# ClashLuke/LocAtE

Measured on AMD Instinct MI355X. Metric: images/sec (G+D step) 64x64 bs=64, higher is better.
Workload: dtype f32 (contractions fp32-faithful on the matrix cores: 2 x scaled fp16 operand pieces / 3 MFMAs per slice where the operand's largest magnitude comes with it, else 3 x bf16 pieces / 6 MFMAs; fp32 accumulate); 1 GPU; LocAtE G+D step, 64x64 RGB, batch 64 per GPU (the fp32 variant - the reference's own precision - of BASELINE.json configs[1]: 64x64 RGB bs 64), self/feature attention at 16x16 and 64x64, random-init weights; global_batch=64, image_size=64, parallelism=dp1, launch=hipGraph replay, G-step generator pass on a second stream

## Files before the change

locate_amd/csrc/conv.hip:

```cpp
#include "igemm.h"



struct PackBatch {
    PackArgs ph[4];
};

__device__ __forceinline__ void pack_tables(const PackArgs& a, int k) {
    int* koff = reinterpret_cast<int*>(a.out + (size_t)a.rows * a.ld);
    unsigned char* ktap = reinterpret_cast<unsigned char*>(koff + a.rows);
    const int T = a.TH * a.TW;
    int off = 0, tap = 31;
    if (k < a.K && T > 0) {
        const int c = k / T, t = k - c * T;
        const int th = t / a.TW, tw = t - th * a.TW;
        off = 4 * (c * a.gHW + (a.dy0 + a.dys * th) * a.gW + a.dx0 + a.dxs * tw - a.dmin);
        tap = t;
    }
    koff[k] = off;
    ktap[k] = (unsigned char)tap;
}

__device__ __forceinline__ void pack_publish_absmax(float m, const PackArgs* phases, int nphase, float* red) {
    m = wave_max(m);
// ... 1704 lines not shown
                                 int scale_group_batch, int scale_stride, const float* bias, float* gx, int64_t gx_bs,
                                 void* workspace, void* counters, int precision, const void* gy_absmax, const void* act_epilogue,
                                 void* stream) {
    const ConvGeom g = make_geom(geom);
    if (int e = geom_check(g, "locate_conv_dgrad")) return e;
    LOCATE_REQUIRE(gy && panel && gx, "locate_conv_dgrad: null pointer");
    return run_igemm(g, 1, gy, gy_bs, panel, scale, scale_group_batch, scale_stride, bias, gx, gx_bs,
                     static_cast<float*>(workspace), static_cast<unsigned*>(counters), precision, static_cast<const unsigned*>(gy_absmax),
                     as_stream(stream), "locate_conv_dgrad", static_cast<const LocateActEpilogue*>(act_epilogue));
}

#define WG_BK 32

struct WgParams {
    const float* x;
    const float* gy;
    float* slab;
    long long x_bs, gy_bs;
    unsigned x_bytes;
    int B, C, H, W, M, OH, OW, KH, KW, stride, pad_h, pad_w;
    int R;
    int N;
    int chunk;
    int zper, Ng;
    unsigned q_mul, ow_mul;
    int q_s1, q_s2, ow_s1, ow_s2;
    int gscale_bg, gscale_stride;
    float* direct_out;
    const float* w_ref;
    const float* inv_scale;
    double* partial;
    const unsigned* x_absmax;
    const unsigned* g_absmax;
};


template <int WGM, int WGN, int TM, int TN>
__device__ __forceinline__ void wgrad_epilogue(const WgParams& p, f32x16 (&acc)[TM][TN], int r0, int m0, int wm, int wn, int lane,
                                               int wid, int tid) {
    const int lrow = lane >> 5, lcol = lane & 31;
    __shared__ double red[4];
    const bool direct = p.direct_out != nullptr;
    float* dst = direct ? p.direct_out : p.slab + (long long)blockIdx.z * p.M * p.R;
    const float sc = (direct && p.inv_scale && p.gscale_bg == 0) ? p.inv_scale[0] : 1.0f;
    double dot = 0.0;
    const bool want_dot = direct && p.w_ref != nullptr;
#pragma unroll
    for (int j = 0; j < TN; ++j) {
        const int r = r0 + (wn * TN + j) * 32 + lcol;
        const bool r_ok = r < p.R;
#pragma unroll
        for (int i = 0; i < TM; ++i) {
            float wref[16];
#pragma unroll
            for (int e = 0; e < 16; ++e) {
                const int m = m0 + (wm * TM + i) * 32 + (e & 3) + 8 * (e >> 2) + 4 * lrow;
                const bool ok = want_dot && r_ok && m < p.M;
                const float* wp_ = ok ? p.w_ref + (long long)m * p.R + r : p.gy;
                wref[e] = ok ? *wp_ : 0.0f;
            }
            float part = 0.0f;
#pragma unroll
            for (int e = 0; e < 16; ++e) {
                const int m = m0 + (wm * TM + i) * 32 + (e & 3) + 8 * (e >> 2) + 4 * lrow;
                const float v = acc[i][j][e];
                part = fmaf(v, wref[e], part);
                if (r_ok && m < p.M) dst[(long long)m * p.R + r] = v * sc;
            }
            dot += (double)part;
        }
    }
    if (direct && p.partial) {
        dot = wave_sum_d(dot);
        if (lane == 0) red[wid] = dot;
        __syncthreads();
        if (tid == 0) p.partial[blockIdx.y * gridDim.x + blockIdx.x] = (red[0] + red[1]) + (red[2] + red[3]);
    }
}

template <int WGM, int WGN, int TM, int TN>
__global__ void __launch_bounds__(256) conv_wgrad_kernel(const WgParams p) {
    constexpr int BM = WGM * TM * 32;
    constexpr int BR = WGN * TN * 32;
    constexpr int G_PT = WG_BK * BM / 256;
    constexpr int X_PT = WG_BK * BR / 256;
    static_assert(WGM * WGN == 4, "four waves");

    __shared__ float Gs[2][WG_BK][BM + 1];
    __shared__ float Xs[2][WG_BK][BR + 1];
    __shared__ int rt_off[BR];
    __shared__ signed char rt_dy[BR], rt_dx[BR];

    const int tid = threadIdx.x, lane = tid & 63, wid = tid >> 6;
    const int wm = wid / WGN, wn = wid % WGN;
    const int r0 = blockIdx.x * BR, m0 = blockIdx.y * BM;
    const int taps = p.KH * p.KW;
    for (int i = tid; i < BR; i += 256) {
        const int r = r0 + i;
        if (r < p.R) {
            const int c = r / taps, t = r - c * taps;
            const int kh = t / p.KW, kw = t - kh * p.KW;
            rt_dy[i] = (signed char)(kh - p.pad_h);
            rt_dx[i] = (signed char)(kw - p.pad_w);
            rt_off[i] = c * p.H * p.W + (kh - p.pad_h) * p.W + (kw - p.pad_w);
        } else {
            rt_dy[i] = rt_dx[i] = 0;
            rt_off[i] = -2147483647 - 1;
        }
    }
    __syncthreads();

    f32x16 acc[TM][TN];
#pragma unroll
    for (int i = 0; i < TM; ++i)
#pragma unroll
        for (int j = 0; j < TN; ++j)
#pragma unroll
            for (int r = 0; r < 16; ++r) acc[i][j][r] = 0.0f;

    const int zgrp = (int)blockIdx.z / p.zper;
    const int n_begin = zgrp * p.Ng + ((int)blockIdx.z - zgrp * p.zper) * p.chunk;
    int n_end = n_begin + p.chunk;
    if (n_end > (zgrp + 1) * p.Ng) n_end = (zgrp + 1) * p.Ng;
    const int nl = tid & 31, sub = tid >> 5;
// ... 54 lines not shown
    auto store_tiles = [&](int buf) {
#pragma unroll
        for (int i = 0; i < G_PT; ++i) Gs[buf][nl][sub + 8 * i] = ((gmask >> i) & 1u) ? greg[i] * gsc : 0.0f;
#pragma unroll
        for (int i = 0; i < X_PT; ++i) Xs[buf][nl][sub + 8 * i] = ((xmask >> i) & 1u) ? xreg[i] : 0.0f;
    };

    const int nsteps = (n_end - n_begin + WG_BK - 1) / WG_BK;
    const int lrow = lane >> 5, lcol = lane & 31;
    if (nsteps > 0) {
        load_tiles(n_begin);
        store_tiles(0);
    }
    __syncthreads();
    for (int s = 0; s < nsteps; ++s) {
        const int buf = s & 1;
        if (s + 1 < nsteps) load_tiles(n_begin + (s + 1) * WG_BK);
#pragma unroll
        for (int k2 = 0; k2 < WG_BK / 2; ++k2) {
            float a[TM], b[TN];
#pragma unroll
            for (int i = 0; i < TM; ++i) a[i] = Gs[buf][k2 * 2 + lrow][(wm * TM + i) * 32 + lcol];
#pragma unroll
            for (int j = 0; j < TN; ++j) b[j] = Xs[buf][k2 * 2 + lrow][(wn * TN + j) * 32 + lcol];
#pragma unroll
            for (int i = 0; i < TM; ++i)
#pragma unroll
                for (int j = 0; j < TN; ++j) acc[i][j] = __builtin_amdgcn_mfma_f32_32x32x2f32(a[i], b[j], acc[i][j], 0, 0, 0);
        }
        if (s + 1 < nsteps) store_tiles(buf ^ 1);
        __syncthreads();
    }

    wgrad_epilogue<WGM, WGN, TM, TN>(p, acc, r0, m0, wm, wn, lane, wid, tid);
}

#define WB_BK 16
#define WB_PITCH 8

template <int WGM, int WGN, int TM, int TN, int NP>
__global__ void __launch_bounds__(256, (WGM * TM > 4 ? 2 : 3)) conv_wgrad_bx6_kernel(const WgParams p) {
    constexpr int BM = WGM * TM * 32;
    constexpr int BR = WGN * TN * 32;
    constexpr int G_PT = BM / 32;
    constexpr int X_PT = BR / 32;
    static_assert(WGM * WGN == 4, "four waves");

    constexpr int NPL = NP == 4 ? 1 : NP;
    __shared__ unsigned Gs[2][NPL][NP == 4 ? 1 : BM][WB_PITCH];
    __shared__ unsigned Xs[2][NPL][NP == 4 ? 1 : BR][WB_PITCH];
    __shared__ __attribute__((aligned(16))) unsigned short G8[2][NP == 4 ? BM : 1][8];
    __shared__ __attribute__((aligned(16))) unsigned short X8[2][NP == 4 ? BR : 1][8];

    const int tid = threadIdx.x, lane = tid & 63, wid = tid >> 6;
    const int wm = wid / WGN, wn = wid % WGN;
    const int r0 = blockIdx.x * BR, m0 = blockIdx.y * BM;
    const int taps = p.KH * p.KW;
    const int np = tid & 7, sub = tid >> 3;
    const int Q = p.OH * p.OW;

    int xoff[X_PT], xdy[X_PT], xdx[X_PT];
#pragma unroll
    for (int i = 0; i < X_PT; ++i) {
        const int r = r0 + sub + 32 * i;
        if (r < p.R) {
            const int c = r / taps, t = r - c * taps;
            const int kh = t / p.KW, kw = t - kh * p.KW;
            xdy[i] = kh - p.pad_h;
            xdx[i] = kw - p.pad_w;
            xoff[i] = 4 * (c * p.H * p.W + xdy[i] * p.W + xdx[i]);
        } else {
            xdy[i] = -(1 << 20);
            xdx[i] = 0;
            xoff[i] = 0;
        }
    }
    const __amdgpu_buffer_rsrc_t xrsrc = __builtin_amdgcn_make_buffer_rsrc(const_cast<float*>(p.x), 0, (int)p.x_bytes, 0x00020000);

    f32x16 acc[TM][TN];
#pragma unroll
    for (int i = 0; i < TM; ++i)
#pragma unroll
        for (int j = 0; j < TN; ++j)
#pragma unroll
            for (int r = 0; r < 16; ++r) acc[i][j][r] = 0.0f;

    const int zgrp = (int)blockIdx.z / p.zper;
    const int n_begin = zgrp * p.Ng + ((int)blockIdx.z - zgrp * p.zper) * p.chunk;
    int n_end = n_begin + p.chunk;
    if (n_end > (zgrp + 1) * p.Ng) n_end = (zgrp + 1) * p.Ng;

    float gs0 = 1.0f, gs1 = 1.0f, gs2 = 1.0f, gs3 = 1.0f, gsc = 1.0f;
    if (p.gscale_bg > 0) {
        const int ng = p.B / p.gscale_bg;
        gs0 = p.inv_scale[0];
        gs1 = ng > 1 ? p.inv_scale[p.gscale_stride] : 1.0f;
        gs2 = ng > 2 ? p.inv_scale[2 * p.gscale_stride] : 1.0f;
        gs3 = ng > 3 ? p.inv_scale[3 * p.gscale_stride] : 1.0f;
    }

    float g_scale = 1.0f, x_scale = 1.0f, g_unscale = 1.0f, x_unscale = 1.0f;
    if constexpr (NP == 2) {
        const float gmax = __uint_as_float(absmax_read(p.g_absmax)) * fmaxf(fmaxf(gs0, gs1), fmaxf(gs2, gs3));
        const int kg_ = f16_scale_exp(__float_as_uint(gmax) + (p.gscale_bg > 0 ? 0x00800000u : 0u));
        const int kx_ = f16_scale_exp(absmax_read(p.x_absmax));
        g_scale = pow2f(kg_); g_unscale = pow2f(-kg_);
        x_scale = pow2f(kx_); x_unscale = pow2f(-kx_);
    }
    if constexpr (NP == 4) {
        const float gmax = __uint_as_float(absmax_read(p.g_absmax)) * fmaxf(fmaxf(gs0, gs1), fmaxf(gs2, gs3));
        const int kg_ = f8_scale_exp(__float_as_uint(gmax) + (p.gscale_bg > 0 ? 0x00800000u : 0u));
        const int kx_ = f8_scale_exp(absmax_read(p.x_absmax));
        g_scale = pow2f(kg_); g_unscale = pow2f(-kg_);
        x_scale = pow2f(kx_); x_unscale = pow2f(-kx_);
    }
    auto q8_pair = [](float v0, float v1) { return (unsigned short)(__builtin_amdgcn_cvt_pk_fp8_f32(v0, v1, 0, false) & 0xffff); };
    auto h8 = [](int row, int pair) { return ((((pair >> 2) ^ (row >> 4)) & 1) << 2) | (pair & 3); };

    float2 greg[G_PT], xreg[X_PT];
    auto load_tiles = [&](int nb) {
        const int n = nb + 2 * np;
        const bool ok = n < n_end;
        const int nn = ok ? n : 0;
        const int b = fastdiv(nn, p.q_mul, p.q_s1, p.q_s2), q = nn - b * Q;
        const int oh = fastdiv(q, p.ow_mul, p.ow_s1, p.ow_s2), ow = q - oh * p.OW;
        const float* gp = p.gy + (long long)b * p.gy_bs + q;
        if (p.gscale_bg > 0) {
            const int bg = p.gscale_bg;
            gsc = gs0;
            gsc = b >= bg ? gs1 : gsc;
            gsc = b >= 2 * bg ? gs2 : gsc;
            gsc = b >= 3 * bg ? gs3 : gsc;
        }
#pragma unroll
        for (int i = 0; i < G_PT; ++i) {
            const int m = m0 + sub + 32 * i;
            const bool v = ok && m < p.M;
            const float2 t = *reinterpret_cast<const float2*>(gp + (v ? (long long)m * Q : 0));
            greg[i] = v ? t : make_float2(0.0f, 0.0f);
        }
        const int iy0 = oh * p.stride, ix0 = ow * p.stride;
        const unsigned base = (unsigned)(4 * ((long long)b * p.x_bs + (long long)iy0 * p.W + ix0));
#pragma unroll
        for (int i = 0; i < X_PT; ++i) {
            const bool vy = ok && (unsigned)(iy0 + xdy[i]) < (unsigned)p.H;
            const bool v0 = vy && (unsigned)(ix0 + xdx[i]) < (unsigned)p.W;
            const bool v1 = vy && (unsigned)(ix0 + p.stride + xdx[i]) < (unsigned)p.W;
            const unsigned o = base + (unsigned)xoff[i];
            xreg[i].x = __builtin_bit_cast(float, __builtin_amdgcn_raw_buffer_load_b32(xrsrc, (int)(v0 ? o : 0x80000000u), 0, 0));
            xreg[i].y = __builtin_bit_cast(float, __builtin_amdgcn_raw_buffer_load_b32(xrsrc, (int)(v1 ? o + 4u * (unsigned)p.stride : 0x80000000u), 0, 0));
        }
    };
    const int wcol = (((np >> 2) ^ ((sub >> 3) & 1)) << 2) | (np & 3);
    auto store_tiles = [&](int buf) {
#pragma unroll
        for (int i = 0; i < G_PT; ++i) {
            if constexpr (NP == 2) {
                unsigned h, l;
                split2_f16_pair(greg[i].x * gsc * g_scale, greg[i].y * gsc * g_scale, h, l);
                Gs[buf][0][sub + 32 * i][wcol] = h;
                Gs[buf][NP - 1][sub + 32 * i][wcol] = l;
            } else if constexpr (NP == 3) {
                unsigned h, m, l;
                split3_trunc_pair(greg[i].x * gsc, greg[i].y * gsc, h, m, l);
                Gs[buf][0][sub + 32 * i][wcol] = h;
                Gs[buf][NP - 2][sub + 32 * i][wcol] = m;
                Gs[buf][NP - 1][sub + 32 * i][wcol] = l;
            } else if constexpr (NP == 4) {
                G8[buf][sub + 32 * i][h8(sub + 32 * i, np)] = q8_pair(greg[i].x * gsc * g_scale, greg[i].y * gsc * g_scale);
            } else {
                Gs[buf][0][sub + 32 * i][wcol] = round_bf16_pair(greg[i].x * gsc, greg[i].y * gsc);
            }
        }
#pragma unroll
        for (int i = 0; i < X_PT; ++i) {
            if constexpr (NP == 2) {
                unsigned h, l;
                split2_f16_pair(xreg[i].x * x_scale, xreg[i].y * x_scale, h, l);
                Xs[buf][0][sub + 32 * i][wcol] = h;
                Xs[buf][NP - 1][sub + 32 * i][wcol] = l;
            } else if constexpr (NP == 3) {
                unsigned h, m, l;
                split3_trunc_pair(xreg[i].x, xreg[i].y, h, m, l);
                Xs[buf][0][sub + 32 * i][wcol] = h;
                Xs[buf][NP - 2][sub + 32 * i][wcol] = m;
                Xs[buf][NP - 1][sub + 32 * i][wcol] = l;
            } else if constexpr (NP == 4) {
                X8[buf][sub + 32 * i][h8(sub + 32 * i, np)] = q8_pair(xreg[i].x * x_scale, xreg[i].y * x_scale);
            } else {
                Xs[buf][0][sub + 32 * i][wcol] = round_bf16_pair(xreg[i].x, xreg[i].y);
            }
        }
    };

    const int nsteps = (n_end - n_begin + WB_BK - 1) / WB_BK;
    const int lrow = lane >> 5, lcol = lane & 31;
    const int rhalf = lrow ^ ((lcol >> 3) & 1);
    if (nsteps > 0) {
        load_tiles(n_begin);
        store_tiles(0);
        load_tiles(n_begin + WB_BK);
    }
    __syncthreads();
    constexpr int PROD = NP == 3 ? 6 : (NP == 2 ? 3 : 1);
    constexpr int NMF = TM * TN * PROD, HALF = NMF / 2;
    using frag_t = typename std::conditional<NP == 2, f16x8, bf16x8>::type;
    for (int s = 0; s < nsteps; ++s) {
        const int buf = s & 1;
        frag_t a[TM][NPL], b[TN][NPL];
        long a8[TM], b8[TN];
        if constexpr (NP == 4) {
            const int half8 = (lrow ^ (lcol >> 4)) & 1;
#pragma unroll
            for (int i = 0; i < TM; ++i) a8[i] = *reinterpret_cast<const long*>(&G8[buf][(wm * TM + i) * 32 + lcol][half8 * 4]);
#pragma unroll
            for (int j = 0; j < TN; ++j) b8[j] = *reinterpret_cast<const long*>(&X8[buf][(wn * TN + j) * 32 + lcol][half8 * 4]);
        } else {
#pragma unroll
            for (int i = 0; i < TM; ++i)
#pragma unroll
                for (int q = 0; q < NPL; ++q) a[i][q] = *reinterpret_cast<const frag_t*>(&Gs[buf][q][(wm * TM + i) * 32 + lcol][rhalf * 4]);
#pragma unroll
            for (int j = 0; j < TN; ++j)
#pragma unroll
                for (int q = 0; q < NPL; ++q) b[j][q] = *reinterpret_cast<const frag_t*>(&Xs[buf][q][(wn * TN + j) * 32 + lcol][rhalf * 4]);
        }
        auto mfmas = [&](int lo, int hi) {
#pragma unroll
            for (int i = 0; i < TM; ++i)
#pragma unroll
                for (int j = 0; j < TN; ++j) {
                    const int base = (i * TN + j) * PROD;
                    if constexpr (NP == 2) {
                        if (base + 0 >= lo && base + 0 < hi) acc[i][j] = __builtin_amdgcn_mfma_f32_32x32x16_f16(a[i][1], b[j][0], acc[i][j], 0, 0, 0);
                        if (base + 1 >= lo && base + 1 < hi) acc[i][j] = __builtin_amdgcn_mfma_f32_32x32x16_f16(a[i][0], b[j][1], acc[i][j], 0, 0, 0);
                        if (base + 2 >= lo && base + 2 < hi) acc[i][j] = __builtin_amdgcn_mfma_f32_32x32x16_f16(a[i][0], b[j][0], acc[i][j], 0, 0, 0);
                    } else if constexpr (NP == 3) {
                        if (base + 0 >= lo && base + 0 < hi) acc[i][j] = __builtin_amdgcn_mfma_f32_32x32x16_bf16(a[i][NP - 1], b[j][0], acc[i][j], 0, 0, 0);
                        if (base + 1 >= lo && base + 1 < hi) acc[i][j] = __builtin_amdgcn_mfma_f32_32x32x16_bf16(a[i][0], b[j][NP - 1], acc[i][j], 0, 0, 0);
                        if (base + 2 >= lo && base + 2 < hi) acc[i][j] = __builtin_amdgcn_mfma_f32_32x32x16_bf16(a[i][NP - 2], b[j][NP - 2], acc[i][j], 0, 0, 0);
                        if (base + 3 >= lo && base + 3 < hi) acc[i][j] = __builtin_amdgcn_mfma_f32_32x32x16_bf16(a[i][NP - 2], b[j][0], acc[i][j], 0, 0, 0);
                        if (base + 4 >= lo && base + 4 < hi) acc[i][j] = __builtin_amdgcn_mfma_f32_32x32x16_bf16(a[i][0], b[j][NP - 2], acc[i][j], 0, 0, 0);
                        if (base + 5 >= lo && base + 5 < hi) acc[i][j] = __builtin_amdgcn_mfma_f32_32x32x16_bf16(a[i][0], b[j][0], acc[i][j], 0, 0, 0);
                    } else if constexpr (NP == 4) {
                        if (base >= lo && base < hi) acc[i][j] = __builtin_amdgcn_mfma_f32_32x32x16_fp8_fp8(a8[i], b8[j], acc[i][j], 0, 0, 0);
                    } else {
                        if (base >= lo && base < hi) acc[i][j] = __builtin_amdgcn_mfma_f32_32x32x16_bf16(a[i][0], b[j][0], acc[i][j], 0, 0, 0);
                    }
                }
        };
        __builtin_amdgcn_sched_barrier(0);
        mfmas(0, HALF);
        __builtin_amdgcn_sched_barrier(0);
        store_tiles(buf ^ 1);
        load_tiles(n_begin + (s + 2) * WB_BK);
        __builtin_amdgcn_sched_barrier(0);
        mfmas(HALF, NMF);
        __syncthreads();
    }
    if constexpr (NP == 2 || NP == 4) {
#pragma unroll
        for (int i = 0; i < TM; ++i)
#pragma unroll
            for (int j = 0; j < TN; ++j)
#pragma unroll
                for (int r = 0; r < 16; ++r) acc[i][j][r] = (acc[i][j][r] * g_unscale) * x_unscale;
    }
    wgrad_epilogue<WGM, WGN, TM, TN>(p, acc, r0, m0, wm, wn, lane, wid, tid);
}

template <int V>
__device__ __forceinline__ void slab_load(const float* p, float (&v)[V]) {
    if constexpr (V == 4) { const float4 t = *reinterpret_cast<const float4*>(p); v[0] = t.x; v[1] = t.y; v[2] = t.z; v[3] = t.w; }
    else v[0] = *p;
}

template <int ZP, int V>
__device__ __forceinline__ void slab_reduce_groups(const float* __restrict__ slab, float* __restrict__ out, int64_t n, int nsplit,
                                                   const float* __restrict__ w_ref, double* __restrict__ partial, int bid, int nblocks,
                                                   int groups, int zper, float* zbuf, double* gscratch) {
    float (*gzsum)[ZP][256 / ZP][V] = reinterpret_cast<float (*)[ZP][256 / ZP][V]>(zbuf);
    constexpr int TPB = 256 / ZP, EPB = TPB * V;
    const int ex = threadIdx.x % TPB, ez = threadIdx.x / TPB;
    const int64_t stride = (int64_t)nblocks * EPB;
    double dot[4] = {0.0, 0.0, 0.0, 0.0};
    for (int64_t i0 = (int64_t)bid * EPB; i0 < n; i0 += stride) {
        const int64_t i = i0 + V * ex;
        float acc[4][V];
#pragma unroll
        for (int k = 0; k < 4; ++k)
#pragma unroll
            for (int e = 0; e < V; ++e) acc[k][e] = 0.0f;
        if (i < n) {
            const float* __restrict__ sp = slab + i;
            for (int z = ez; z < nsplit; z += 8 * ZP) {
                float v[8][V];
#pragma unroll
                for (int q = 0; q < 8; ++q) {
                    if (z + q * ZP < nsplit) slab_load<V>(sp + (int64_t)(z + q * ZP) * n, v[q]);
                    else
#pragma unroll
// ... 780 lines not shown
        LOCATE_REQUIRE(r.x && r.gy && r.gw && r.grid_x > 0 && r.M > 0 && r.C > 0 && r.N > 0, "locate_wgrad_batch: bad record");
        b.r[i].block0 = (int)blocks;
        blocks += (long long)r.grid_x * ((r.M + skw_mt(r.M) - 1) / skw_mt(r.M));
    }
    LOCATE_REQUIRE(blocks < (1ll << 31), "locate_wgrad_batch: too many blocks");
    skinny_wgrad_batch_kernel<<<(unsigned)blocks, 256, 0, as_stream(stream)>>>(b, n);
    LOCATE_LAUNCH_CHECK("locate_wgrad_batch");
    return LOCATE_OK;
}

static bool wgrad_group_dots_ok(const ConvGeom& g, int groups) {
    if (groups < 2 || groups > 4 || g.B % groups != 0 || skinny_wgrad_ok(g) || onepix_wgrad_ok(g)) return false;
    const PwPlan q = pw_plan(g, groups);
    if (q.ok) return q.zper > 0;
    return (long long)g.B * g.OH * g.OW < (1ll << 31);
}
LOCATE_API int locate_conv_wgrad_group_partials(const int* geom, int groups) {
    const ConvGeom g = make_geom(geom);
    if (geom_check(g, "locate_conv_wgrad_group_partials") || !wgrad_group_dots_ok(g, groups)) return 0;
    const PwPlan q = pw_plan(g, groups);
    if (q.ok) return wgrad_reduce_grid((int64_t)g.M * g.C, q.nslab);
    int bm, nsplit, chunk, tiles;
    wgrad_plan(g, &bm, &nsplit, &chunk, &tiles, groups);
    return wgrad_reduce_grid((int64_t)g.M * g.C * g.KH * g.KW, nsplit);
}
LOCATE_API size_t locate_conv_wgrad_group_workspace_bytes(const int* geom, int groups) {
    const ConvGeom g = make_geom(geom);
    if (geom_check(g, "locate_conv_wgrad_group_workspace_bytes") || !wgrad_group_dots_ok(g, groups)) return 0;
    const PwPlan q = pw_plan(g, groups);
    if (q.ok) return (size_t)q.nslab * g.M * g.C * sizeof(float);
    int bm, nsplit, chunk, tiles;
    wgrad_plan(g, &bm, &nsplit, &chunk, &tiles, groups);
    return (size_t)nsplit * g.M * g.C * g.KH * g.KW * sizeof(float);
}

LOCATE_API int locate_conv_wgrad(const int* geom, const float* x, int64_t x_bs, const float* gy, int64_t gy_bs, float* gw,
                                 const float* w_ref, const float* inv_scale, int scale_group_batch, int scale_stride,
                                 double* inner_partial, void* workspace, int precision, const void* x_absmax, const void* gy_absmax,
                                 void* deferred_reduce, void* stream) {
    const ConvGeom g = make_geom(geom);
    if (int e = geom_check(g, "locate_conv_wgrad")) return e;
    LOCATE_REQUIRE(precision >= 0 && precision <= 3, "locate_conv_wgrad: precision must be 0 (fp32-faithful, bf16 pieces), 1 (bf16 operands), 2 (fp32-faithful, fp16 pieces) or 3 (fp8 operands)");
    LOCATE_REQUIRE(precision < 2 || (x_absmax && gy_absmax), "locate_conv_wgrad: precisions 2 and 3 need the absmax words of x and gy");
    LOCATE_REQUIRE(x && gy && gw, "locate_conv_wgrad: null pointer");
    LOCATE_REQUIRE(!inner_partial || w_ref, "locate_conv_wgrad: inner_partial needs w_ref");
    const int gd = (scale_group_batch > 0 && w_ref && inner_partial && g.B % scale_group_batch == 0) ? g.B / scale_group_batch : 0;
    LOCATE_REQUIRE(scale_group_batch >= 0 && (scale_group_batch == 0 || (inv_scale && g.B % scale_group_batch == 0 &&
                   g.B / scale_group_batch <= 4 && ((!w_ref && !inner_partial) || wgrad_group_dots_ok(g, gd)))),
                   "locate_conv_wgrad: bad group scaling arguments (per-call partials: see locate_conv_wgrad_group_partials)");
    hipStream_t st = as_stream(stream);
    if (deferred_reduce) memset(deferred_reduce, 0, sizeof(SlabRec));
    auto reduce = [&](const float* slab, int64_t n, int nsplit, const float* scale, int zper, const char* who) -> int {
        const int rg = wgrad_reduce_grid(n, nsplit);
        const int zp = wgrad_reduce_zp(nsplit, n);
        if (deferred_reduce) {
            SlabRec r;
            r.slab = slab; r.out = gw; r.w_ref = w_ref; r.inv_scale = scale; r.partial = inner_partial;
            r.n = n; r.nsplit = nsplit; r.zp = zp; r.grid = rg; r.block0 = 0; r.groups = gd; r.zper = zper;
            memcpy(deferred_reduce, &r, sizeof(r));
            return LOCATE_OK;
        }
        if (zp == 16) slab_reduce_kernel<16><<<rg, 256, 0, st>>>(slab, gw, n, nsplit, w_ref, scale, inner_partial, gd, zper);
        else if (zp == 4) slab_reduce_kernel<4><<<rg, 256, 0, st>>>(slab, gw, n, nsplit, w_ref, scale, inner_partial, gd, zper);
        else slab_reduce_kernel<1><<<rg, 256, 0, st>>>(slab, gw, n, nsplit, w_ref, scale, inner_partial, gd, zper);
        LOCATE_LAUNCH_CHECK(who);
        return LOCATE_OK;
// ... 42 lines not shown
            else if (key == 1) pw_wgrad_kernel<1, 2, 3><<<grid, 256, 0, st>>>(q);
            else if (key == 2) pw_wgrad_kernel<2, 1, 3><<<grid, 256, 0, st>>>(q);
            else pw_wgrad_kernel<2, 2, 3><<<grid, 256, 0, st>>>(q);
        }
        LOCATE_LAUNCH_CHECK("locate_conv_wgrad(pointwise)");
        return reduce(q.slab, (int64_t)g.M * g.C, pq.nslab, grouped ? nullptr : inv_scale, pq.zper, "locate_conv_wgrad(pointwise reduce)");
    }
    int bm, nsplit, chunk, tiles, zper;
    wgrad_plan(g, &bm, &nsplit, &chunk, &tiles, gd, &zper);
    LOCATE_REQUIRE(nsplit == 1 || workspace, "locate_conv_wgrad: split reduction needs a workspace");
    WgParams p;
    p.x = x; p.gy = gy; p.slab = static_cast<float*>(workspace); p.x_bs = x_bs; p.gy_bs = gy_bs;
    p.B = g.B; p.C = g.C; p.H = g.H; p.W = g.W; p.M = g.M; p.OH = g.OH; p.OW = g.OW; p.KH = g.KH; p.KW = g.KW;
    p.stride = g.stride; p.pad_h = g.pad_h; p.pad_w = g.pad_w;
    p.R = g.C * g.KH * g.KW; p.N = g.B * g.OH * g.OW; p.chunk = chunk;
    p.zper = zper; p.Ng = gd > 1 ? p.N / gd : p.N;
    fastdiv_make((unsigned)(g.OH * g.OW), &p.q_mul, &p.q_s1, &p.q_s2);
    fastdiv_make((unsigned)g.OW, &p.ow_mul, &p.ow_s1, &p.ow_s2);
    const bool direct = nsplit == 1;
    const bool grouped = scale_group_batch > 0;
    p.gscale_bg = scale_group_batch; p.gscale_stride = scale_stride;
    p.x_absmax = static_cast<const unsigned*>(x_absmax);
    p.g_absmax = static_cast<const unsigned*>(gy_absmax);
    p.direct_out = direct ? gw : nullptr;
    p.w_ref = direct ? w_ref : nullptr;
    p.inv_scale = (direct || grouped) ? inv_scale : nullptr;
    p.partial = direct ? inner_partial : nullptr;
    dim3 grid((p.R + 127) / 128, (g.M + bm - 1) / bm, nsplit);
    const long long x_extent = 4ll * ((long long)(g.B - 1) * x_bs + (long long)g.C * g.H * g.W);
    p.x_bytes = (unsigned)x_extent;
    const bool pairs_ok = ((g.OH * g.OW) & 1) == 0 && (g.OW & 1) == 0 && (gy_bs & 1) == 0 && (chunk & 1) == 0 &&
                          (reinterpret_cast<uintptr_t>(gy) & 7) == 0 && x_extent > 0 && x_extent < (1ll << 31) - (1 << 20);
    LOCATE_REQUIRE(bm != 192 || pairs_ok, "locate_conv_wgrad: layers with M %% 192 == 0 on even maps take the paired-load kernels - gy must be 8-byte aligned with an even batch stride");
    if (precision == 3 && pairs_ok) {
        if (bm == 192) conv_wgrad_bx6_kernel<2, 2, 3, 2, 4><<<grid, 256, 0, st>>>(p);
        else if (bm == 128) conv_wgrad_bx6_kernel<2, 2, 2, 2, 4><<<grid, 256, 0, st>>>(p);
        else if (bm == 96) conv_wgrad_bx6_kernel<1, 4, 3, 1, 4><<<grid, 256, 0, st>>>(p);
        else if (bm == 64) conv_wgrad_bx6_kernel<1, 4, 2, 1, 4><<<grid, 256, 0, st>>>(p);
        else conv_wgrad_bx6_kernel<1, 4, 1, 1, 4><<<grid, 256, 0, st>>>(p);
    } else if (pairs_ok && precision == 1) {
        if (bm == 192) conv_wgrad_bx6_kernel<2, 2, 3, 2, 1><<<grid, 256, 0, st>>>(p);
        else if (bm == 128) conv_wgrad_bx6_kernel<2, 2, 2, 2, 1><<<grid, 256, 0, st>>>(p);
        else if (bm == 96) conv_wgrad_bx6_kernel<1, 4, 3, 1, 1><<<grid, 256, 0, st>>>(p);
        else if (bm == 64) conv_wgrad_bx6_kernel<1, 4, 2, 1, 1><<<grid, 256, 0, st>>>(p);
        else conv_wgrad_bx6_kernel<1, 4, 1, 1, 1><<<grid, 256, 0, st>>>(p);
    } else if (pairs_ok && precision == 2 && !path_disabled("wbx6")) {
        if (bm == 192) conv_wgrad_bx6_kernel<2, 2, 3, 2, 2><<<grid, 256, 0, st>>>(p);
        else if (bm == 128) conv_wgrad_bx6_kernel<2, 2, 2, 2, 2><<<grid, 256, 0, st>>>(p);
        else if (bm == 96) conv_wgrad_bx6_kernel<1, 4, 3, 1, 2><<<grid, 256, 0, st>>>(p);
        else if (bm == 64) conv_wgrad_bx6_kernel<1, 4, 2, 1, 2><<<grid, 256, 0, st>>>(p);
        else conv_wgrad_bx6_kernel<1, 4, 1, 1, 2><<<grid, 256, 0, st>>>(p);
    } else if (pairs_ok && !path_disabled("wbx6")) {
        if (bm == 192) conv_wgrad_bx6_kernel<2, 2, 3, 2, 3><<<grid, 256, 0, st>>>(p);
        else if (bm == 128) conv_wgrad_bx6_kernel<2, 2, 2, 2, 3><<<grid, 256, 0, st>>>(p);
        else if (bm == 96) conv_wgrad_bx6_kernel<1, 4, 3, 1, 3><<<grid, 256, 0, st>>>(p);
        else if (bm == 64) conv_wgrad_bx6_kernel<1, 4, 2, 1, 3><<<grid, 256, 0, st>>>(p);
        else conv_wgrad_bx6_kernel<1, 4, 1, 1, 3><<<grid, 256, 0, st>>>(p);
    } else if (bm == 128) conv_wgrad_kernel<2, 2, 2, 2><<<grid, 256, 0, st>>>(p);
    else if (bm == 96) conv_wgrad_kernel<1, 4, 3, 1><<<grid, 256, 0, st>>>(p);
    else if (bm == 64) conv_wgrad_kernel<1, 4, 2, 1><<<grid, 256, 0, st>>>(p);
    else conv_wgrad_kernel<1, 4, 1, 1><<<grid, 256, 0, st>>>(p);
    LOCATE_LAUNCH_CHECK("locate_conv_wgrad(gemm)");
    if (!direct) return reduce(p.slab, (int64_t)g.M * p.R, nsplit, grouped ? nullptr : inv_scale, zper, "locate_conv_wgrad(reduce)");
    return LOCATE_OK;
}

LOCATE_API size_t locate_slab_reduce_record_bytes(void) { return sizeof(SlabRec); }
LOCATE_API int locate_slab_reduce_max(void) { return SLAB_MAX; }
LOCATE_API int locate_slab_reduce_record_blocks(const void* record) {
    if (!record) return 0;
    SlabRec r;
    memcpy(&r, record, sizeof(r));
    return r.grid;
}
LOCATE_API int locate_slab_reduce_batch(const void* records, int n, void* stream) {
    LOCATE_REQUIRE(records && n > 0 && n <= SLAB_MAX, "locate_slab_reduce_batch: 1 .. locate_slab_reduce_max() records");
    SlabBatch b;
    memcpy(b.r, records, (size_t)n * sizeof(SlabRec));
    long long blocks = 0;
    for (int i = 0; i < n; ++i) {
        const SlabRec& r = b.r[i];
        LOCATE_REQUIRE(r.slab && r.out && r.n > 0 && r.nsplit > 0 && r.grid > 0 && (r.zp == 1 || r.zp == 4 || r.zp == 16),
                       "locate_slab_reduce_batch: bad record");
        b.r[i].block0 = (int)blocks;
        blocks += r.grid;
    }
    slab_reduce_batch_kernel<<<(unsigned)blocks, 256, 0, as_stream(stream)>>>(b, n);
    LOCATE_LAUNCH_CHECK("locate_slab_reduce_batch");
    return LOCATE_OK;
}
// ... 1 lines not shown
```

Measured before the change: 7306 images/sec.

## Deepen wgrad bx6 stage to two K-slices with quad loads and XCD tile order

The paired-load weight-gradient kernel can now process two 16-wide K slices per stage (KS=2) when using fp16 split operands (NP=2). It loads gy as float4 quads with incrementally advanced per-group addresses instead of recomputing fastdiv each step, and interleaves fragment reads, loads and MFMAs with sched_group_barrier hints. Block indices are remapped through xcd_tile so neighbouring tiles land on the same XCD for L2 reuse. Shared memory is unified into one buffer and the occupancy bound is computed from LDS use. The deeper stage is enabled only for bm=192, so wider tiles trade more LDS and registers per block for fewer barriers per K.

```diff
diff --git a/locate_amd/csrc/conv.hip b/locate_amd/csrc/conv.hip
--- a/locate_amd/csrc/conv.hip
+++ b/locate_amd/csrc/conv.hip
@@ -1760,16 +1760,16 @@
     double* partial;
     const unsigned* x_absmax;
     const unsigned* g_absmax;
+    int xcd_order;
 };
 
 
 template <int WGM, int WGN, int TM, int TN>
 __device__ __forceinline__ void wgrad_epilogue(const WgParams& p, f32x16 (&acc)[TM][TN], int r0, int m0, int wm, int wn, int lane,
-                                               int wid, int tid) {
+                                               int wid, int tid, int bx, int by, int bz, double* red) {
     const int lrow = lane >> 5, lcol = lane & 31;
-    __shared__ double red[4];
     const bool direct = p.direct_out != nullptr;
-    float* dst = direct ? p.direct_out : p.slab + (long long)blockIdx.z * p.M * p.R;
+    float* dst = direct ? p.direct_out : p.slab + (long long)bz * p.M * p.R;
     const float sc = (direct && p.inv_scale && p.gscale_bg == 0) ? p.inv_scale[0] : 1.0f;
     double dot = 0.0;
     const bool want_dot = direct && p.w_ref != nullptr;
@@ -1802,7 +1802,7 @@
         dot = wave_sum_d(dot);
         if (lane == 0) red[wid] = dot;
         __syncthreads();
-        if (tid == 0) p.partial[blockIdx.y * gridDim.x + blockIdx.x] = (red[0] + red[1]) + (red[2] + red[3]);
+        if (tid == 0) p.partial[by * (int)gridDim.x + bx] = (red[0] + red[1]) + (red[2] + red[3]);
     }
 }
 
@@ -1818,6 +1818,7 @@
     __shared__ float Xs[2][WG_BK][BR + 1];
     __shared__ int rt_off[BR];
     __shared__ signed char rt_dy[BR], rt_dx[BR];
+    __shared__ double red[4];
 
     const int tid = threadIdx.x, lane = tid & 63, wid = tid >> 6;
     const int wm = wid / WGN, wn = wid % WGN;
@@ -1938,29 +1939,43 @@
         __syncthreads();
     }
 
-    wgrad_epilogue<WGM, WGN, TM, TN>(p, acc, r0, m0, wm, wn, lane, wid, tid);
+    wgrad_epilogue<WGM, WGN, TM, TN>(p, acc, r0, m0, wm, wn, lane, wid, tid, blockIdx.x, blockIdx.y, blockIdx.z, red);
 }
 
 #define WB_BK 16
 #define WB_PITCH 8
 
-template <int WGM, int WGN, int TM, int TN, int NP>
-__global__ void __launch_bounds__(256, (WGM * TM > 4 ? 2 : 3)) conv_wgrad_bx6_kernel(const WgParams p) {
+constexpr int wgrad_bx6_waves(int bm, int br, int np, int ks) {
+    return bm > 128 ? 2 : (3 * (2 * (np == 4 ? 16 : np * 32 * ks) * (bm + br)) > 160 * 1024 ? 2 : 3);
+}
+template <int WGM, int WGN, int TM, int TN, int NP, int KS = 1, bool QUAD = false>
+__global__ void __launch_bounds__(256, wgrad_bx6_waves(WGM * TM * 32, WGN * TN * 32, NP, KS)) conv_wgrad_bx6_kernel(const WgParams p) {
     constexpr int BM = WGM * TM * 32;
     constexpr int BR = WGN * TN * 32;
     constexpr int G_PT = BM / 32;
     constexpr int X_PT = BR / 32;
     static_assert(WGM * WGN == 4, "four waves");
+    static_assert(KS == 1 || (KS == 2 && NP != 4), "one or two slices per stage; fp8 rows hold one slice");
+    static_assert(!QUAD || KS == 2, "eight quads span two slices");
+    constexpr int BKS = WB_BK * KS;
+    constexpr int VEC = QUAD ? 4 : 2;
+    constexpr int NG = BKS / (8 * VEC);
+    constexpr int PITCH = WB_PITCH * KS;
 
     constexpr int NPL = NP == 4 ? 1 : NP;
-    __shared__ unsigned Gs[2][NPL][NP == 4 ? 1 : BM][WB_PITCH];
-    __shared__ unsigned Xs[2][NPL][NP == 4 ? 1 : BR][WB_PITCH];
-    __shared__ __attribute__((aligned(16))) unsigned short G8[2][NP == 4 ? BM : 1][8];
-    __shared__ __attribute__((aligned(16))) unsigned short X8[2][NP == 4 ? BR : 1][8];
+    constexpr int G_DW = NP == 4 ? 2 * BM * 4 : 2 * NPL * BM * PITCH;
+    constexpr int X_DW = NP == 4 ? 2 * BR * 4 : 2 * NPL * BR * PITCH;
+    __shared__ __attribute__((aligned(16))) unsigned smem[G_DW + X_DW];
+    unsigned (*const Gs)[NPL][BM][PITCH] = reinterpret_cast<unsigned (*)[NPL][BM][PITCH]>(smem);
+    unsigned (*const Xs)[NPL][BR][PITCH] = reinterpret_cast<unsigned (*)[NPL][BR][PITCH]>(smem + G_DW);
+    unsigned short (*const G8)[BM][8] = reinterpret_cast<unsigned short (*)[BM][8]>(smem);
+    unsigned short (*const X8)[BR][8] = reinterpret_cast<unsigned short (*)[BR][8]>(smem + G_DW);
 
     const int tid = threadIdx.x, lane = tid & 63, wid = tid >> 6;
     const int wm = wid / WGN, wn = wid % WGN;
-    const int r0 = blockIdx.x * BR, m0 = blockIdx.y * BM;
+    int bx = blockIdx.x, by = blockIdx.y, bz = blockIdx.z;
+    if (p.xcd_order) xcd_tile(bx, by, bz);
+    const int r0 = bx * BR, m0 = by * BM;
     const int taps = p.KH * p.KW;
     const int np = tid & 7, sub = tid >> 3;
     const int Q = p.OH * p.OW;
@@ -1991,12 +2006,14 @@
 #pragma unroll
             for (int r = 0; r < 16; ++r) acc[i][j][r] = 0.0f;
 
-    const int zgrp = (int)blockIdx.z / p.zper;
-    const int n_begin = zgrp * p.Ng + ((int)blockIdx.z - zgrp * p.zper) * p.chunk;
+    const int zgrp = bz / p.zper;
+    const int n_begin = zgrp * p.Ng + (bz - zgrp * p.zper) * p.chunk;
     int n_end = n_begin + p.chunk;
     if (n_end > (zgrp + 1) * p.Ng) n_end = (zgrp + 1) * p.Ng;
 
-    float gs0 = 1.0f, gs1 = 1.0f, gs2 = 1.0f, gs3 = 1.0f, gsc = 1.0f;
+    float gs0 = 1.0f, gs1 = 1.0f, gs2 = 1.0f, gs3 = 1.0f, gsc[NG];
+#pragma unroll
+    for (int g = 0; g < NG; ++g) gsc[g] = 1.0f;
     if (p.gscale_bg > 0) {
         const int ng = p.B / p.gscale_bg;
         gs0 = p.inv_scale[0];
@@ -2023,89 +2040,186 @@
     auto q8_pair = [](float v0, float v1) { return (unsigned short)(__builtin_amdgcn_cvt_pk_fp8_f32(v0, v1, 0, false) & 0xffff); };
     auto h8 = [](int row, int pair) { return ((((pair >> 2) ^ (row >> 4)) & 1) << 2) | (pair & 3); };
 
-    float2 greg[G_PT], xreg[X_PT];
-    auto load_tiles = [&](int nb) {
-        const int n = nb + 2 * np;
-        const bool ok = n < n_end;
-        const int nn = ok ? n : 0;
+    const int st_db = fastdiv(BKS, p.q_mul, p.q_s1, p.q_s2), st_rem = BKS - st_db * Q;
+    const int st_doh = fastdiv(st_rem, p.ow_mul, p.ow_s1, p.ow_s2), st_dow = st_rem - st_doh * p.OW;
+    const int st_dy = st_doh * p.stride, st_dx = st_dow * p.stride, lim_y = p.OH * p.stride, lim_x = p.OW * p.stride;
+    const long long gstep = (long long)st_db * p.gy_bs + st_rem, gwrap = p.gy_bs - Q;
+    const unsigned xstep = 4u * (unsigned)((long long)st_db * p.x_bs + (long long)st_dy * p.W + st_dx);
+    const unsigned xrow = 4u * (unsigned)(p.stride * p.W - lim_x);
+    const unsigned ximg = 4u * (unsigned)(p.x_bs - (long long)lim_y * p.W);
+    int pn[NG], pb[NG], piy[NG], pix[NG];
+    long long pg[NG];
+    unsigned pxb[NG];
+#pragma unroll
+    for (int g = 0; g < (KS == 1 ? 0 : NG); ++g) {
+        const int n = n_begin + 16 * g + VEC * np;
+        const int nn = n < n_end ? n : 0;
         const int b = fastdiv(nn, p.q_mul, p.q_s1, p.q_s2), q = nn - b * Q;
         const int oh = fastdiv(q, p.ow_mul, p.ow_s1, p.ow_s2), ow = q - oh * p.OW;
-        const float* gp = p.gy + (long long)b * p.gy_bs + q;
-        if (p.gscale_bg > 0) {
-            const int bg = p.gscale_bg;
-            gsc = gs0;
-            gsc = b >= bg ? gs1 : gsc;
-            gsc = b >= 2 * bg ? gs2 : gsc;
-            gsc = b >= 3 * bg ? gs3 : gsc;
-        }
-#pragma unroll
-        for (int i = 0; i < G_PT; ++i) {
-            const int m = m0 + sub + 32 * i;
-            const bool v = ok && m < p.M;
-            const float2 t = *reinterpret_cast<const float2*>(gp + (v ? (long long)m * Q : 0));
-            greg[i] = v ? t : make_float2(0.0f, 0.0f);
-        }
-        const int iy0 = oh * p.stride, ix0 = ow * p.stride;
-        const unsigned base = (unsigned)(4 * ((long long)b * p.x_bs + (long long)iy0 * p.W + ix0));
-#pragma unroll
-        for (int i = 0; i < X_PT; ++i) {
-            const bool vy = ok && (unsigned)(iy0 + xdy[i]) < (unsigned)p.H;
-            const bool v0 = vy && (unsigned)(ix0 + xdx[i]) < (unsigned)p.W;
-            const bool v1 = vy && (unsigned)(ix0 + p.stride + xdx[i]) < (unsigned)p.W;
-            const unsigned o = base + (unsigned)xoff[i];
-            xreg[i].x = __builtin_bit_cast(float, __builtin_amdgcn_raw_buffer_load_b32(xrsrc, (int)(v0 ? o : 0x80000000u), 0, 0));
-            xreg[i].y = __builtin_bit_cast(float, __builtin_amdgcn_raw_buffer_load_b32(xrsrc, (int)(v1 ? o + 4u * (unsigned)p.stride : 0x80000000u), 0, 0));
+        pn[g] = n; pb[g] = b; piy[g] = oh * p.stride; pix[g] = ow * p.stride;
+        pg[g] = (long long)b * p.gy_bs + q;
+        pxb[g] = (unsigned)(4 * ((long long)b * p.x_bs + (long long)piy[g] * p.W + pix[g]));
+    }
+
+    float greg[G_PT][NG * VEC], xreg[X_PT][NG * VEC];
+    int ld_n = n_begin;
+    auto load_tiles = [&]() {
+        if constexpr (KS == 1) {
+            const int n = ld_n + 2 * np;
+            ld_n += BKS;
+            const bool ok = n < n_end;
+            const int nn = ok ? n : 0;
+            const int b = fastdiv(nn, p.q_mul, p.q_s1, p.q_s2), q = nn - b * Q;
+            const int oh = fastdiv(q, p.ow_mul, p.ow_s1, p.ow_s2), ow = q - oh * p.OW;
+            const float* gp = p.gy + (long long)b * p.gy_bs + q;
+            if (p.gscale_bg > 0) {
+                const int bg = p.gscale_bg;
+                gsc[0] = gs0;
+                gsc[0] = b >= bg ? gs1 : gsc[0];
+                gsc[0] = b >= 2 * bg ? gs2 : gsc[0];
+                gsc[0] = b >= 3 * bg ? gs3 : gsc[0];
+            }
+#pragma unroll
+            for (int i = 0; i < G_PT; ++i) {
+                const int m = m0 + sub + 32 * i;
+                const bool v = ok && m < p.M;
+                const float2 t = *reinterpret_cast<const float2*>(gp + (v ? (long long)m * Q : 0));
+                greg[i][0] = v ? t.x : 0.0f; greg[i][1] = v ? t.y : 0.0f;
+            }
+            const int iy0 = oh * p.stride, ix0 = ow * p.stride;
+            const unsigned base = (unsigned)(4 * ((long long)b * p.x_bs + (long long)iy0 * p.W + ix0));
+#pragma unroll
+            for (int i = 0; i < X_PT; ++i) {
+                const bool vy = ok && (unsigned)(iy0 + xdy[i]) < (unsigned)p.H;
+                const bool v0 = vy && (unsigned)(ix0 + xdx[i]) < (unsigned)p.W;
+                const bool v1 = vy && (unsigned)(ix0 + p.stride + xdx[i]) < (unsigned)p.W;
+                const unsigned o = base + (unsigned)xoff[i];
+                xreg[i][0] = __builtin_bit_cast(float, __builtin_amdgcn_raw_buffer_load_b32(xrsrc, (int)(v0 ? o : 0x80000000u), 0, 0));
+                xreg[i][1] = __builtin_bit_cast(float, __builtin_amdgcn_raw_buffer_load_b32(xrsrc, (int)(v1 ? o + 4u * (unsigned)p.stride : 0x80000000u), 0, 0));
+            }
+            return;
+        }
+#pragma unroll
+        for (int g = 0; g < NG; ++g) {
+            const bool ok = pn[g] < n_end;
+            if (p.gscale_bg > 0) {
+                const int bg = p.gscale_bg, b = pb[g];
+                gsc[g] = gs0;
+                gsc[g] = b >= bg ? gs1 : gsc[g];
+                gsc[g] = b >= 2 * bg ? gs2 : gsc[g];
+                gsc[g] = b >= 3 * bg ? gs3 : gsc[g];
+            }
+#pragma unroll
+            for (int i = 0; i < G_PT; ++i) {
+                const int m = m0 + sub + 32 * i;
+                const bool v = ok & (m < p.M);
+                const float* gp = p.gy + (v ? pg[g] + (long long)m * Q : 0);
+                if constexpr (QUAD) {
+                    const float4 t = *reinterpret_cast<const float4*>(gp);
+                    greg[i][0] = v ? t.x : 0.0f; greg[i][1] = v ? t.y : 0.0f; greg[i][2] = v ? t.z : 0.0f; greg[i][3] = v ? t.w : 0.0f;
+                } else {
+                    const float2 t = *reinterpret_cast<const float2*>(gp);
+                    greg[i][2 * g] = v ? t.x : 0.0f; greg[i][2 * g + 1] = v ? t.y : 0.0f;
+                }
+            }
+            const int iy0 = piy[g], ix0 = pix[g];
+#pragma unroll
+            for (int i = 0; i < X_PT; ++i) {
+                const bool vy = ok & ((unsigned)(iy0 + xdy[i]) < (unsigned)p.H);
+                const unsigned o = pxb[g] + (unsigned)xoff[i];
+#pragma unroll
+                for (int e = 0; e < VEC; ++e) {
+                    const bool ve = vy & ((unsigned)(ix0 + e * p.stride + xdx[i]) < (unsigned)p.W);
+                    xreg[i][VEC * g + e] = __builtin_bit_cast(float, __builtin_amdgcn_raw_buffer_load_b32(xrsrc, (int)((o + 4u * (unsigned)(e * p.stride)) | ((ve ? 0u : 1u) << 31)), 0, 0));
+                }
+            }
+            int ix = ix0 + st_dx;
+            const bool cx = ix >= lim_x;
+            ix -= cx ? lim_x : 0;
+            int iy = iy0 + st_dy + (cx ? p.stride : 0);
+            const bool cy = iy >= lim_y;
+            iy -= cy ? lim_y : 0;
+            pix[g] = ix; piy[g] = iy;
+            pb[g] += st_db + (cy ? 1 : 0);
+            pn[g] += BKS;
+            pg[g] += gstep + (cy ? gwrap : 0);
+            pxb[g] += xstep + (cx ? xrow : 0u) + (cy ? ximg : 0u);
         }
     };
-    const int wcol = (((np >> 2) ^ ((sub >> 3) & 1)) << 2) | (np & 3);
+    const int wsw = KS == 2 ? ((((sub >> 2) & 1) << 1) | ((sub >> 3) & 1)) : ((sub >> 3) & 1);
+    int wcol[NG];
+#pragma unroll
+    for (int g = 0; g < NG; ++g)
+        wcol[g] = QUAD ? ((((np >> 1) ^ wsw) << 2) | ((np & 1) << 1)) : ((((KS == 2 ? 2 * g : 0) + (np >> 2)) ^ wsw) << 2) | (np & 3);
+    auto put = [](unsigned* row, int col, unsigned v0, unsigned v1) {
+        if constexpr (QUAD) *reinterpret_cast<uint2*>(row + col) = make_uint2(v0, v1);
+        else row[col] = v0;
+    };
     auto store_tiles = [&](int buf) {
 #pragma unroll
-        for (int i = 0; i < G_PT; ++i) {
-            if constexpr (NP == 2) {
-                unsigned h, l;
-                split2_f16_pair(greg[i].x * gsc * g_scale, greg[i].y * gsc * g_scale, h, l);
-                Gs[buf][0][sub + 32 * i][wcol] = h;
-                Gs[buf][NP - 1][sub + 32 * i][wcol] = l;
-            } else if constexpr (NP == 3) {
-                unsigned h, m, l;
-                split3_trunc_pair(greg[i].x * gsc, greg[i].y * gsc, h, m, l);
-                Gs[buf][0][sub + 32 * i][wcol] = h;
-                Gs[buf][NP - 2][sub + 32 * i][wcol] = m;
-                Gs[buf][NP - 1][sub + 32 * i][wcol] = l;
-            } else if constexpr (NP == 4) {
-                G8[buf][sub + 32 * i][h8(sub + 32 * i, np)] = q8_pair(greg[i].x * gsc * g_scale, greg[i].y * gsc * g_scale);
-            } else {
-                Gs[buf][0][sub + 32 * i][wcol] = round_bf16_pair(greg[i].x * gsc, greg[i].y * gsc);
-            }
-        }
-#pragma unroll
-        for (int i = 0; i < X_PT; ++i) {
-            if constexpr (NP == 2) {
-                unsigned h, l;
-                split2_f16_pair(xreg[i].x * x_scale, xreg[i].y * x_scale, h, l);
-                Xs[buf][0][sub + 32 * i][wcol] = h;
-                Xs[buf][NP - 1][sub + 32 * i][wcol] = l;
-            } else if constexpr (NP == 3) {
-                unsigned h, m, l;
-                split3_trunc_pair(xreg[i].x, xreg[i].y, h, m, l);
-                Xs[buf][0][sub + 32 * i][wcol] = h;
-                Xs[buf][NP - 2][sub + 32 * i][wcol] = m;
-                Xs[buf][NP - 1][sub + 32 * i][wcol] = l;
-            } else if constexpr (NP == 4) {
-                X8[buf][sub + 32 * i][h8(sub + 32 * i, np)] = q8_pair(xreg[i].x * x_scale, xreg[i].y * x_scale);
-            } else {
-                Xs[buf][0][sub + 32 * i][wcol] = round_bf16_pair(xreg[i].x, xreg[i].y);
+        for (int g = 0; g < NG; ++g) {
+#pragma unroll
+            for (int i = 0; i < G_PT; ++i) {
+                const int row = sub + 32 * i;
+                const float (&v_)[NG * VEC] = greg[i]; const int e0 = QUAD ? 0 : 2 * g;
+                if constexpr (NP == 2) {
+                    unsigned h0, l0, h1 = 0, l1 = 0;
+                    split2_f16_pair(v_[e0] * gsc[g] * g_scale, v_[e0 + 1] * gsc[g] * g_scale, h0, l0);
+                    if constexpr (QUAD) split2_f16_pair(v_[2] * gsc[g] * g_scale, v_[3] * gsc[g] * g_scale, h1, l1);
+                    put(Gs[buf][0][row], wcol[g], h0, h1);
+                    put(Gs[buf][NP - 1][row], wcol[g], l0, l1);
+                } else if constexpr (NP == 3) {
+                    unsigned h0, m0_, l0, h1 = 0, m1_ = 0, l1 = 0;
+                    split3_trunc_pair(v_[e0] * gsc[g], v_[e0 + 1] * gsc[g], h0, m0_, l0);
+                    if constexpr (QUAD) split3_trunc_pair(v_[2] * gsc[g], v_[3] * gsc[g], h1, m1_, l1);
+                    put(Gs[buf][0][row], wcol[g], h0, h1);
+                    put(Gs[buf][NP - 2][row], wcol[g], m0_, m1_);
+                    put(Gs[buf][NP - 1][row], wcol[g], l0, l1);
+                } else if constexpr (NP == 4) {
+                    G8[buf][row][h8(row, np)] = q8_pair(v_[e0] * gsc[g] * g_scale, v_[e0 + 1] * gsc[g] * g_scale);
+                } else {
+                    const unsigned h0 = round_bf16_pair(v_[e0] * gsc[g], v_[e0 + 1] * gsc[g]);
+                    unsigned h1 = 0;
+                    if constexpr (QUAD) h1 = round_bf16_pair(v_[2] * gsc[g], v_[3] * gsc[g]);
+                    put(Gs[buf][0][row], wcol[g], h0, h1);
+                }
+            }
+#pragma unroll
+            for (int i = 0; i < X_PT; ++i) {
+                const int row = sub + 32 * i;
+                const float (&v_)[NG * VEC] = xreg[i]; const int e0 = QUAD ? 0 : 2 * g;
+                if constexpr (NP == 2) {
+                    unsigned h0, l0, h1 = 0, l1 = 0;
+                    split2_f16_pair(v_[e0] * x_scale, v_[e0 + 1] * x_scale, h0, l0);
+                    if constexpr (QUAD) split2_f16_pair(v_[2] * x_scale, v_[3] * x_scale, h1, l1);
+                    put(Xs[buf][0][row], wcol[g], h0, h1);
+                    put(Xs[buf][NP - 1][row], wcol[g], l0, l1);
+                } else if constexpr (NP == 3) {
+                    unsigned h0, m0_, l0, h1 = 0, m1_ = 0, l1 = 0;
+                    split3_trunc_pair(v_[e0], v_[e0 + 1], h0, m0_, l0);
+                    if constexpr (QUAD) split3_trunc_pair(v_[2], v_[3], h1, m1_, l1);
+                    put(Xs[buf][0][row], wcol[g], h0, h1);
+                    put(Xs[buf][NP - 2][row], wcol[g], m0_, m1_);
+                    put(Xs[buf][NP - 1][row], wcol[g], l0, l1);
+                } else if constexpr (NP == 4) {
+                    X8[buf][row][h8(row, np)] = q8_pair(v_[e0] * x_scale, v_[e0 + 1] * x_scale);
+                } else {
+                    const unsigned h0 = round_bf16_pair(v_[e0], v_[e0 + 1]);
+                    unsigned h1 = 0;
+                    if constexpr (QUAD) h1 = round_bf16_pair(v_[2], v_[3]);
+                    put(Xs[buf][0][row], wcol[g], h0, h1);
+                }
             }
         }
     };
 
-    const int nsteps = (n_end - n_begin + WB_BK - 1) / WB_BK;
+    const int nsteps = (n_end - n_begin + BKS - 1) / BKS;
     const int lrow = lane >> 5, lcol = lane & 31;
-    const int rhalf = lrow ^ ((lcol >> 3) & 1);
+    const int rsw = KS == 2 ? ((((lcol >> 2) & 1) << 1) | ((lcol >> 3) & 1)) : ((lcol >> 3) & 1);
     if (nsteps > 0) {
-        load_tiles(n_begin);
+        load_tiles();
         store_tiles(0);
-        load_tiles(n_begin + WB_BK);
+        load_tiles();
     }
     __syncthreads();
     constexpr int PROD = NP == 3 ? 6 : (NP == 2 ? 3 : 1);
@@ -2115,6 +2229,17 @@
         const int buf = s & 1;
         frag_t a[TM][NPL], b[TN][NPL];
         long a8[TM], b8[TN];
+        auto fragments = [&](int sl) {
+            const int fcol = (((KS == 2 ? 2 * sl : 0) + lrow) ^ rsw) << 2;
+#pragma unroll
+            for (int i = 0; i < TM; ++i)
+#pragma unroll
+                for (int q = 0; q < NPL; ++q) a[i][q] = *reinterpret_cast<const frag_t*>(&Gs[buf][q][(wm * TM + i) * 32 + lcol][fcol]);
+#pragma unroll
+            for (int j = 0; j < TN; ++j)
+#pragma unroll
+                for (int q = 0; q < NPL; ++q) b[j][q] = *reinterpret_cast<const frag_t*>(&Xs[buf][q][(wn * TN + j) * 32 + lcol][fcol]);
+        };
         if constexpr (NP == 4) {
             const int half8 = (lrow ^ (lcol >> 4)) & 1;
 #pragma unroll
@@ -2122,14 +2247,7 @@
 #pragma unroll
             for (int j = 0; j < TN; ++j) b8[j] = *reinterpret_cast<const long*>(&X8[buf][(wn * TN + j) * 32 + lcol][half8 * 4]);
         } else {
-#pragma unroll
-            for (int i = 0; i < TM; ++i)
-#pragma unroll
-                for (int q = 0; q < NPL; ++q) a[i][q] = *reinterpret_cast<const frag_t*>(&Gs[buf][q][(wm * TM + i) * 32 + lcol][rhalf * 4]);
-#pragma unroll
-            for (int j = 0; j < TN; ++j)
-#pragma unroll
-                for (int q = 0; q < NPL; ++q) b[j][q] = *reinterpret_cast<const frag_t*>(&Xs[buf][q][(wn * TN + j) * 32 + lcol][rhalf * 4]);
+            fragments(0);
         }
         auto mfmas = [&](int lo, int hi) {
 #pragma unroll
@@ -2156,12 +2274,25 @@
                 }
         };
         __builtin_amdgcn_sched_barrier(0);
-        mfmas(0, HALF);
+        mfmas(0, KS == 2 ? NMF : HALF);
         __builtin_amdgcn_sched_barrier(0);
         store_tiles(buf ^ 1);
-        load_tiles(n_begin + (s + 2) * WB_BK);
-        __builtin_amdgcn_sched_barrier(0);
-        mfmas(HALF, NMF);
+        if constexpr (KS == 1) {
+            load_tiles();
+            __builtin_amdgcn_sched_barrier(0);
+            mfmas(HALF, NMF);
+        } else {
+            __builtin_amdgcn_sched_barrier(0);
+            load_tiles();
+            fragments(1);
+            mfmas(0, NMF);
+#pragma unroll
+            for (int k = 0; k < NMF; ++k) {
+                __builtin_amdgcn_sched_group_barrier(0x008, 1, 0);
+                __builtin_amdgcn_sched_group_barrier(0x020, 1, 0);
+                __builtin_amdgcn_sched_group_barrier(0x002, 3, 0);
+            }
+        }
         __syncthreads();
     }
     if constexpr (NP == 2 || NP == 4) {
@@ -2172,7 +2303,7 @@
 #pragma unroll
                 for (int r = 0; r < 16; ++r) acc[i][j][r] = (acc[i][j][r] * g_unscale) * x_unscale;
     }
-    wgrad_epilogue<WGM, WGN, TM, TN>(p, acc, r0, m0, wm, wn, lane, wid, tid);
+    wgrad_epilogue<WGM, WGN, TM, TN>(p, acc, r0, m0, wm, wn, lane, wid, tid, bx, by, bz, reinterpret_cast<double*>(smem));
 }
 
 template <int V>
@@ -3019,6 +3150,26 @@
     int bm, nsplit, chunk, tiles;
     wgrad_plan(g, &bm, &nsplit, &chunk, &tiles, groups);
     return (size_t)nsplit * g.M * g.C * g.KH * g.KW * sizeof(float);
+}
+
+static int wgrad_stage_slices(int bm, int np) {
+    if (np != 2) return 1;
+    switch (bm) {
+    case 192: return 2;
+    case 128: return 1;
+    case 96: return 1;
+    case 64: return 1;
+    default: return 1;
+    }
+}
+
+template <int NP, int KS, bool QUAD>
+static void launch_wgrad_bx6(int bm, dim3 grid, hipStream_t st, const WgParams& p) {
+    if (bm == 192) conv_wgrad_bx6_kernel<2, 2, 3, 2, NP, KS, QUAD><<<grid, 256, 0, st>>>(p);
+    else if (bm == 128) conv_wgrad_bx6_kernel<2, 2, 2, 2, NP, KS, QUAD><<<grid, 256, 0, st>>>(p);
+    else if (bm == 96) conv_wgrad_bx6_kernel<1, 4, 3, 1, NP, KS, QUAD><<<grid, 256, 0, st>>>(p);
+    else if (bm == 64) conv_wgrad_bx6_kernel<1, 4, 2, 1, NP, KS, QUAD><<<grid, 256, 0, st>>>(p);
+    else conv_wgrad_bx6_kernel<1, 4, 1, 1, NP, KS, QUAD><<<grid, 256, 0, st>>>(p);
 }
 
 LOCATE_API int locate_conv_wgrad(const int* geom, const float* x, int64_t x_bs, const float* gy, int64_t gy_bs, float* gw,
@@ -3127,30 +3278,29 @@
     const bool pairs_ok = ((g.OH * g.OW) & 1) == 0 && (g.OW & 1) == 0 && (gy_bs & 1) == 0 && (chunk & 1) == 0 &&
                           (reinterpret_cast<uintptr_t>(gy) & 7) == 0 && x_extent > 0 && x_extent < (1ll << 31) - (1 << 20);
     LOCATE_REQUIRE(bm != 192 || pairs_ok, "locate_conv_wgrad: layers with M %% 192 == 0 on even maps take the paired-load kernels - gy must be 8-byte aligned with an even batch stride");
+    const bool quads_ok = pairs_ok && (g.OW & 3) == 0 && ((g.OH * g.OW) & 3) == 0 && (gy_bs & 3) == 0 && (chunk & 3) == 0 &&
+                          (reinterpret_cast<uintptr_t>(gy) & 15) == 0;
+    p.xcd_order = path_disabled("wgxcd") ? 0 : 1;
+    const int np = precision == 3 ? 4 : (precision == 1 ? 1 : (precision == 2 ? 2 : 3));
+    int ks = path_disabled("wg32") ? 1 : wgrad_stage_slices(bm, np);
+    bool quad = ks == 2 && quads_ok && !path_disabled("wgquad");
+#ifndef LOCATE_DEBUG_KNOBS
+    if (!quad) ks = 1;
+#else
+    if (!quad && !path_disabled("wgquad")) ks = 1;
+#endif
     if (precision == 3 && pairs_ok) {
-        if (bm == 192) conv_wgrad_bx6_kernel<2, 2, 3, 2, 4><<<grid, 256, 0, st>>>(p);
-        else if (bm == 128) conv_wgrad_bx6_kernel<2, 2, 2, 2, 4><<<grid, 256, 0, st>>>(p);
-        else if (bm == 96) conv_wgrad_bx6_kernel<1, 4, 3, 1, 4><<<grid, 256, 0, st>>>(p);
-        else if (bm == 64) conv_wgrad_bx6_kernel<1, 4, 2, 1, 4><<<grid, 256, 0, st>>>(p);
-        else conv_wgrad_bx6_kernel<1, 4, 1, 1, 4><<<grid, 256, 0, st>>>(p);
+        launch_wgrad_bx6<4, 1, false>(bm, grid, st, p);
     } else if (pairs_ok && precision == 1) {
-        if (bm == 192) conv_wgrad_bx6_kernel<2, 2, 3, 2, 1><<<grid, 256, 0, st>>>(p);
-        else if (bm == 128) conv_wgrad_bx6_kernel<2, 2, 2, 2, 1><<<grid, 256, 0, st>>>(p);
-        else if (bm == 96) conv_wgrad_bx6_kernel<1, 4, 3, 1, 1><<<grid, 256, 0, st>>>(p);
-        else if (bm == 64) conv_wgrad_bx6_kernel<1, 4, 2, 1, 1><<<grid, 256, 0, st>>>(p);
-        else conv_wgrad_bx6_kernel<1, 4, 1, 1, 1><<<grid, 256, 0, st>>>(p);
+        launch_wgrad_bx6<1, 1, false>(bm, grid, st, p);
     } else if (pairs_ok && precision == 2 && !path_disabled("wbx6")) {
-        if (bm == 192) conv_wgrad_bx6_kernel<2, 2, 3, 2, 2><<<grid, 256, 0, st>>>(p);
-        else if (bm == 128) conv_wgrad_bx6_kernel<2, 2, 2, 2, 2><<<grid, 256, 0, st>>>(p);
-        else if (bm == 96) conv_wgrad_bx6_kernel<1, 4, 3, 1, 2><<<grid, 256, 0, st>>>(p);
-        else if (bm == 64) conv_wgrad_bx6_kernel<1, 4, 2, 1, 2><<<grid, 256, 0, st>>>(p);
-        else conv_wgrad_bx6_kernel<1, 4, 1, 1, 2><<<grid, 256, 0, st>>>(p);
+        if (quad) launch_wgrad_bx6<2, 2, true>(bm, grid, st, p);
+#ifdef LOCATE_DEBUG_KNOBS
+        else if (ks == 2) launch_wgrad_bx6<2, 2, false>(bm, grid, st, p);
+#endif
+        else launch_wgrad_bx6<2, 1, false>(bm, grid, st, p);
     } else if (pairs_ok && !path_disabled("wbx6")) {
-        if (bm == 192) conv_wgrad_bx6_kernel<2, 2, 3, 2, 3><<<grid, 256, 0, st>>>(p);
-        else if (bm == 128) conv_wgrad_bx6_kernel<2, 2, 2, 2, 3><<<grid, 256, 0, st>>>(p);
-        else if (bm == 96) conv_wgrad_bx6_kernel<1, 4, 3, 1, 3><<<grid, 256, 0, st>>>(p);
-        else if (bm == 64) conv_wgrad_bx6_kernel<1, 4, 2, 1, 3><<<grid, 256, 0, st>>>(p);
-        else conv_wgrad_bx6_kernel<1, 4, 1, 1, 3><<<grid, 256, 0, st>>>(p);
+        launch_wgrad_bx6<3, 1, false>(bm, grid, st, p);
     } else if (bm == 128) conv_wgrad_kernel<2, 2, 2, 2><<<grid, 256, 0, st>>>(p);
     else if (bm == 96) conv_wgrad_kernel<1, 4, 3, 1><<<grid, 256, 0, st>>>(p);
     else if (bm == 64) conv_wgrad_kernel<1, 4, 2, 1><<<grid, 256, 0, st>>>(p);
```

New measurement: 7316 images/sec, median of 2. Within noise of the previous version (+0.1%).
